# Shimly-2/DRL-on-robot-arm

Hardware: AMD Instinct MI355X
Metric: env-steps/sec at N parallel envs (rl_reach_env) (higher is better)
Workload: dtype f64

## Files before the change

### drl-on-robot-arm_amd/csrc/armenv_learner.h

```cpp
#pragma once
#include <hip/hip_runtime.h>
#include <stdint.h>

#include "armenv_math.h"

namespace armenv {
namespace learner {

constexpr int LRN_H = 256;
constexpr int LRN_A = 3;
constexpr int LRN_TM = 64, LRN_TN = 64, LRN_TK = 16;
constexpr int LRN_KSPLIT = 256;
constexpr int LRN_MAX_GEMMS = 6;
constexpr int LRN_MAX_TENSORS = 12;

struct Feat {
  const float *p0, *p1;
  int ld0, ld1, split, nf, aug;
  int64_t rows;
};

AE_DEV float feat_at(const Feat &F, int64_t r, int f) {
  if (r >= F.rows) return 0.f;
  if (f < F.split) return F.p0[r * F.ld0 + f];
  if (f < F.nf) return F.p1[r * F.ld1 + (f - F.split)];
  return (F.aug && f == F.nf) ? 1.f : 0.f;
}

enum { EPI_STORE = 0,
       EPI_BIAS_RELU = 1,
       EPI_MASK = 2,
       EPI_DRELU_W = 3 };

struct Gemm {
  Feat a, b;
  int ta, tb;
  int M, N;
  int64_t K, kchunk;
  int splits, tiles_m, tiles_n, first_block;
  float *C;
  int ldc;
  int64_t split_stride;
  int epi;
  const float *bias, *mask, *w;
  int ldm;
  float scale;
};

struct GemmList {
  Gemm g[LRN_MAX_GEMMS];
  int n;
};


AE_DEV float wave_sum(float x) {
#pragma unroll
  for (int o = 32; o >= 1; o >>= 1) x += __shfl_xor(x, o, 64);
  return x;
}

AE_DEV float4 row4(const float *p, int64_t b, int lane) { return reinterpret_cast<const float4 *>(p + b * LRN_H)[lane]; }
AE_DEV float dot4(float4 a, float4 b) { return a.x * b.x + a.y * b.y + a.z * b.z + a.w * b.w; }

AE_DEV void box_muller(uint32_t w0, uint32_t w1, float &z0, float &z1) {
  const float u1 = (float)((w0 >> 8) + 1u) * (1.0f / 16777216.0f);
  const float u2 = (float)(w1 >> 8) * (1.0f / 16777216.0f);
  const float r = sqrtf(-2.0f * logf(u1));
  float sn, cs;
  sincosf(6.283185307179586f * u2, &sn, &cs);
  z0 = r * cs;
  z1 = r * sn;
}


AE_DEV void head3(const float *h2, const float *W3, const float *b3, int64_t b, int lane, float (&u)[LRN_A]) {
  const float4 h = row4(h2, b, lane);
#pragma unroll
  for (int j = 0; j < LRN_A; ++j) u[j] = wave_sum(dot4(h, row4(W3, j, lane))) + b3[j];
}

AE_DEV float head1(float4 h, float4 w, const float *b3) { return wave_sum(dot4(h, w)) + b3[0]; }
AE_DEV float head1(const float *h2, const float *W3, const float *b3, int64_t b, int lane) {
  return head1(row4(h2, b, lane), row4(W3, 0, lane), b3);
}

AE_DEV void row_noise(const float *noise, uint64_t seed, uint64_t draw, float policy_noise, float noise_clip, int64_t b,
                      float (&nz)[LRN_A]) {
  float z[4];
  if (noise) {
#pragma unroll
    for (int j = 0; j < LRN_A; ++j) z[j] = noise[b * LRN_A + j];
  } else {
    uint32_t c[4] = {(uint32_t)b, (uint32_t)((uint64_t)b >> 32), (uint32_t)draw, (uint32_t)(draw >> 32)};
    philox4x32_10(c, (uint32_t)seed, (uint32_t)(seed >> 32));
    box_muller(c[0], c[1], z[0], z[1]);
    box_muller(c[2], c[3], z[2], z[3]);
  }
#pragma unroll
  for (int j = 0; j < LRN_A; ++j) nz[j] = fminf(fmaxf(z[j] * policy_noise, -noise_clip), noise_clip);
}

AE_DEV float proposal(float u, float nz, float bound) {
  const float v = tanhf(u) * bound + nz;
  return fminf(fmaxf(v, -bound), bound);
}

AE_DEV void store_action(const float (&u)[LRN_A], float bound, float *a, float *tanh_out, bool keep_tanh, int64_t b) {
#pragma unroll
  for (int j = 0; j < LRN_A; ++j) {
    const float th = tanhf(u[j]);
    if (keep_tanh) tanh_out[b * LRN_A + j] = th;
    a[b * LRN_A + j] = th * bound;
  }
}

AE_DEV void store_d2(float4 h, float4 w, float d3, float *d2, int64_t b, int lane) {
  float4 d;
  d.x = h.x > 0.f ? d3 * w.x : 0.f;
  d.y = h.y > 0.f ? d3 * w.y : 0.f;
  d.z = h.z > 0.f ? d3 * w.z : 0.f;
  d.w = h.w > 0.f ? d3 * w.w : 0.f;
  reinterpret_cast<float4 *>(d2 + b * LRN_H)[lane] = d;
}

struct ActorHeadArgs {
  int64_t B;
  const float *t_h2, *t_W3, *t_b3, *noise;
  uint64_t seed, draw;
  float bound, policy_noise, noise_clip;
  float *a2;
  int with_actor;
  const float *h2, *W3, *b3;
  float *a, *tanh_out;
};


struct CriticHeadArgs {
  int64_t B;
  float gamma, inv_b;
  const float *rewards;
  const uint8_t *dones;
  const float *t_h2[2], *t_W3[2], *t_b3[2];
  const float *h2[2], *W3[2], *b3[2];
  float *d3[2];
  float *d2[2];
  float *loss_rows;
};


struct DaddpgActorHeadArgs {
  int64_t B;
  float bound;
  const float *h2[3], *W3[3], *b3[3];
  float *a[3];
  float *tanh_out;
};

struct DaddpgCriticHeadArgs {
  int64_t B;
  float gamma, inv_b;
  const float *rewards;
  const uint8_t *dones;
  const float *t_h2[2];
  const float *t_W3, *t_b3;
  const float *h2, *W3, *b3;
  float *d3;
  float *d2;
  float *loss_rows;
};

struct Datd3ActorHeadArgs {
  int64_t B;
  float bound, policy_noise, noise_clip;
  const float *noise;
  uint64_t seed, draw;
  const float *t_h2[2], *t_W3[2], *t_b3[2];
  float *a2[2];
  const float *h2, *W3, *b3;
  float *a, *tanh_out;
};

struct Datd3CriticHeadArgs {
  int64_t B;
  float gamma, inv_b;
  int darc;
  float w_min, w_max, reg;
  const float *rewards;
  const uint8_t *dones;
  const float *t_h2[2], *t_W3[2], *t_b3[2];
  const float *h2, *W3, *b3;
  const float *o_h2, *o_W3, *o_b3;
  float *d3;
  float *d2;
  float *loss_rows;
};

struct ActorBackArgs {
  int64_t B;
  int in_dim;
  int state_dim;
  float bound;
  const float *dc1;
  const float *Wq1;
  const float *tanh_a;
  const float *h2, *W3;
  float *du;
  float *da2;
};


struct AdamTensor {
  float *p, *m, *v, *tp;
  const float *partial;
  int rows, cols, ldp, c0;
  int first;
};

struct AdamArgs {
  AdamTensor t[LRN_MAX_TENSORS];
  int n, total, splits;
  int64_t split_stride;
  float step_size, bc2_sqrt, beta1, beta2, eps, tau;
  int soft;
  const float *loss_rows;
  int loss_cols;
  float loss_w1;
  int64_t B;
  float inv_b;
  float *loss;
};


struct GemmStride {
  int64_t a0, a1, b0, b1;
  int64_t C, bias, mask, w;
};

struct GemmStrideList {
  GemmStride g[LRN_MAX_GEMMS];
};

struct HeadStride {
  int64_t ws, W3, b3, rows, noise;
};

struct ActorBackStride {
  int64_t ws, Wq1, W3;
};

#define LRN_POP 0
#include "armenv_learner_kernels.inc"
#undef LRN_POP
#define LRN_POP 1
#include "armenv_learner_kernels.inc"
#undef LRN_POP

}
}
```

### drl-on-robot-arm_amd/csrc/armenv_learner_kernels.inc

```
#if LRN_POP
#define LRN_KERNEL(name) name##_pop_kernel
#define LRN_POP_PARAM(decl) , decl
#define LRN_MEMBER(ptr, stride) ((ptr) + (int64_t)blockIdx.y * (stride))
#else
#define LRN_KERNEL(name) name##_kernel
#define LRN_POP_PARAM(decl)
#define LRN_MEMBER(ptr, stride) ptr
#endif

__global__ __launch_bounds__(256) void LRN_KERNEL(gemm)(GemmList L LRN_POP_PARAM(GemmStrideList S)) {
  __shared__ float As[LRN_TK][LRN_TM + 4];
  __shared__ float Bs[LRN_TK][LRN_TN + 4];
  int pi = 0;
  while (pi + 1 < L.n && (int)blockIdx.x >= L.g[pi + 1].first_block) ++pi;
#if LRN_POP
  Gemm G = L.g[pi];
  {
    const GemmStride &T = S.g[pi];
    const int64_t p = blockIdx.y;
    G.a.p0 += p * T.a0; G.a.p1 += p * T.a1;
    G.b.p0 += p * T.b0; G.b.p1 += p * T.b1;
    G.C += p * T.C; G.bias += p * T.bias; G.mask += p * T.mask; G.w += p * T.w;
  }
#else
  const Gemm &G = L.g[pi];
#endif
  int t = (int)blockIdx.x - G.first_block;
  const int tn = t % G.tiles_n;
  t /= G.tiles_n;
  const int tm = t % G.tiles_m;
  const int s = t / G.tiles_m;
  const int m0 = tm * LRN_TM, n0 = tn * LRN_TN;
  const int64_t kbeg = (int64_t)s * G.kchunk;
  const int64_t kend = kbeg + G.kchunk < G.K ? kbeg + G.kchunk : G.K;
  const int tid = threadIdx.x, lane = tid & 63, wave = tid >> 6;
  const int wm = (wave & 1) * 32, wn = (wave >> 1) * 32;
  typedef float f32x16 __attribute__((ext_vector_type(16)));
  f32x16 acc;
#pragma unroll
  for (int r = 0; r < 16; ++r) acc[r] = 0.f;

  for (int64_t k0 = kbeg; k0 < kend; k0 += LRN_TK) {
#pragma unroll
    for (int i = 0; i < LRN_TM * LRN_TK / 256; ++i) {
      const int e = tid + 256 * i;
      int mm, kk;
      if (G.ta) { mm = e % LRN_TM; kk = e / LRN_TM; } else { kk = e % LRN_TK; mm = e / LRN_TK; }
      const int64_t k = k0 + kk;
      float v = 0.f;
      if (k < kend) v = G.ta ? feat_at(G.a, k, m0 + mm) : feat_at(G.a, m0 + mm, (int)k);
      As[kk][mm] = v;
    }
#pragma unroll
    for (int i = 0; i < LRN_TN * LRN_TK / 256; ++i) {
      const int e = tid + 256 * i;
      int nn, kk;
      if (G.tb) { kk = e % LRN_TK; nn = e / LRN_TK; } else { nn = e % LRN_TN; kk = e / LRN_TN; }
      const int64_t k = k0 + kk;
      float v = 0.f;
      if (k < kend) v = G.tb ? feat_at(G.b, n0 + nn, (int)k) : feat_at(G.b, k, n0 + nn);
      Bs[kk][nn] = v;
    }
    __syncthreads();
#pragma unroll
    for (int kk = 0; kk < LRN_TK; kk += 2) {
      const float av = As[kk + (lane >> 5)][wm + (lane & 31)];
      const float bv = Bs[kk + (lane >> 5)][wn + (lane & 31)];
      acc = __builtin_amdgcn_mfma_f32_32x32x2f32(av, bv, acc, 0, 0, 0);
    }
    __syncthreads();
  }

  float *C = G.C + (int64_t)s * G.split_stride;
  const int n = n0 + wn + (lane & 31);
  if (n >= G.N) return;
#pragma unroll
  for (int r = 0; r < 16; ++r) {
    const int m = m0 + wm + (r & 3) + 8 * (r >> 2) + 4 * (lane >> 5);
    if (m >= G.M) continue;
    float v = acc[r];
    if (G.epi == EPI_BIAS_RELU) {
      v = v + G.bias[n];
      v = v > 0.f ? v : 0.f;
    } else if (G.epi == EPI_MASK) {
      v = G.mask[(int64_t)m * G.ldm + n] > 0.f ? v : 0.f;
    } else if (G.epi == EPI_DRELU_W) {
      v = (v + G.bias[n] > 0.f) ? G.scale * G.w[n] : 0.f;
    }
    C[(int64_t)m * G.ldc + n] = v;
  }
}

__global__ __launch_bounds__(256) void LRN_KERNEL(actor_head)(ActorHeadArgs P LRN_POP_PARAM(HeadStride S)) {
#if LRN_POP
  {
    const int64_t p = blockIdx.y;
    P.t_h2 += p * S.ws; P.a2 += p * S.ws; P.h2 += p * S.ws; P.a += p * S.ws; P.tanh_out += p * S.ws;
    P.t_W3 += p * S.W3; P.W3 += p * S.W3; P.t_b3 += p * S.b3; P.b3 += p * S.b3;
    if (P.noise) P.noise += p * S.noise;
    P.seed += (uint64_t)p;
  }
#endif
  const int lane = threadIdx.x & 63;
  const int64_t nb = (P.B + 3) / 4;
  const bool actor = (int64_t)blockIdx.x >= nb;
  const int64_t b = ((int64_t)blockIdx.x - (actor ? nb : 0)) * 4 + (threadIdx.x >> 6);
  if (b >= P.B) return;
  float u[LRN_A];
  head3(actor ? P.h2 : P.t_h2, actor ? P.W3 : P.t_W3, actor ? P.b3 : P.t_b3, b, lane, u);
  if (lane != 0) return;
  if (actor) {
    store_action(u, P.bound, P.a, P.tanh_out, true, b);
    return;
  }
  float nz[LRN_A];
  row_noise(P.noise, P.seed, P.draw, P.policy_noise, P.noise_clip, b, nz);
#pragma unroll
  for (int j = 0; j < LRN_A; ++j) P.a2[b * LRN_A + j] = proposal(u[j], nz[j], P.bound);
}

__global__ __launch_bounds__(256) void LRN_KERNEL(critic_head)(CriticHeadArgs P LRN_POP_PARAM(HeadStride S)) {
#if LRN_POP
  {
    const int64_t p = blockIdx.y;
    P.rewards += p * S.rows; P.dones += p * S.rows; P.loss_rows += p * S.ws;
#pragma unroll
    for (int i = 0; i < 2; ++i) {
      P.t_h2[i] += p * S.ws; P.h2[i] += p * S.ws; P.d3[i] += p * S.ws; P.d2[i] += p * S.ws;
      P.t_W3[i] += p * S.W3; P.W3[i] += p * S.W3; P.t_b3[i] += p * S.b3; P.b3[i] += p * S.b3;
    }
  }
#endif
  const int lane = threadIdx.x & 63;
  const int64_t b = (int64_t)blockIdx.x * 4 + (threadIdx.x >> 6);
  if (b >= P.B) return;
  float tq[2], q[2];
#pragma unroll
  for (int i = 0; i < 2; ++i) {
    tq[i] = head1(P.t_h2[i], P.t_W3[i], P.t_b3[i], b, lane);
    q[i] = head1(P.h2[i], P.W3[i], P.b3[i], b, lane);
  }
  const float notdone = 1.0f - (P.dones[b] ? 1.0f : 0.0f);
  const float target = P.rewards[b] + notdone * P.gamma * fminf(tq[0], tq[1]);
#pragma unroll
  for (int i = 0; i < 2; ++i) {
    const float e = q[i] - target;
    const float d3 = 2.0f * e * P.inv_b;
    if (lane == 0) {
      P.d3[i][b] = d3;
      P.loss_rows[2 * b + i] = e * e;
    }
    store_d2(row4(P.h2[i], b, lane), row4(P.W3[i], 0, lane), d3, P.d2[i], b, lane);
  }
}

__global__ __launch_bounds__(256) void LRN_KERNEL(daddpg_actor_head)(DaddpgActorHeadArgs P LRN_POP_PARAM(HeadStride S)) {
  const int lane = threadIdx.x & 63;
  const int64_t nb = (P.B + 3) / 4;
  const int k = (int)((int64_t)blockIdx.x / nb);
  const int64_t b = ((int64_t)blockIdx.x - k * nb) * 4 + (threadIdx.x >> 6);
  if (k > 2 || b >= P.B) return;
  float u[LRN_A];
  head3(LRN_MEMBER(P.h2[k], S.ws), LRN_MEMBER(P.W3[k], S.W3), LRN_MEMBER(P.b3[k], S.b3), b, lane, u);
  if (lane != 0) return;
  store_action(u, P.bound, LRN_MEMBER(P.a[k], S.ws), LRN_MEMBER(P.tanh_out, S.ws), k == 2, b);
}

__global__ __launch_bounds__(256) void LRN_KERNEL(daddpg_critic_head)(DaddpgCriticHeadArgs P LRN_POP_PARAM(HeadStride S)) {
#if LRN_POP
  {
    const int64_t p = blockIdx.y;
    P.rewards += p * S.rows; P.dones += p * S.rows;
    P.t_h2[0] += p * S.ws; P.t_h2[1] += p * S.ws; P.h2 += p * S.ws; P.d3 += p * S.ws; P.d2 += p * S.ws; P.loss_rows += p * S.ws;
    P.t_W3 += p * S.W3; P.W3 += p * S.W3; P.t_b3 += p * S.b3; P.b3 += p * S.b3;
  }
#endif
  const int lane = threadIdx.x & 63;
  const int64_t b = (int64_t)blockIdx.x * 4 + (threadIdx.x >> 6);
  if (b >= P.B) return;
  const float4 tw = row4(P.t_W3, 0, lane);
  const float tq0 = head1(row4(P.t_h2[0], b, lane), tw, P.t_b3);
  const float tq1 = head1(row4(P.t_h2[1], b, lane), tw, P.t_b3);
  const float4 h = row4(P.h2, b, lane), w = row4(P.W3, 0, lane);
  const float q = head1(h, w, P.b3);
  const float notdone = 1.0f - (P.dones[b] ? 1.0f : 0.0f);
  const float target = P.rewards[b] + notdone * P.gamma * fminf(tq0, tq1);
  const float e = q - target;
  const float d3 = 2.0f * e * P.inv_b;
  if (lane == 0) {
    P.d3[b] = d3;
    P.loss_rows[b] = e * e;
  }
  store_d2(h, w, d3, P.d2, b, lane);
}

__global__ __launch_bounds__(256) void LRN_KERNEL(datd3_actor_head)(Datd3ActorHeadArgs P LRN_POP_PARAM(HeadStride S)) {
#if LRN_POP
  {
    const int64_t p = blockIdx.y;
#pragma unroll
    for (int i = 0; i < 2; ++i) { P.t_h2[i] += p * S.ws; P.a2[i] += p * S.ws; P.t_W3[i] += p * S.W3; P.t_b3[i] += p * S.b3; }
    P.h2 += p * S.ws; P.a += p * S.ws; P.tanh_out += p * S.ws; P.W3 += p * S.W3; P.b3 += p * S.b3;
    if (P.noise) P.noise += p * S.noise;
    P.seed += (uint64_t)p;
  }
#endif
  const int lane = threadIdx.x & 63;
  const int64_t nb = (P.B + 3) / 4;
  const bool actor = (int64_t)blockIdx.x >= nb;
  const int64_t b = ((int64_t)blockIdx.x - (actor ? nb : 0)) * 4 + (threadIdx.x >> 6);
  if (b >= P.B) return;
  if (actor) {
    float u[LRN_A];
    head3(P.h2, P.W3, P.b3, b, lane, u);
    if (lane != 0) return;
    store_action(u, P.bound, P.a, P.tanh_out, true, b);
    return;
  }
  float u[2][LRN_A];
#pragma unroll
  for (int i = 0; i < 2; ++i) head3(P.t_h2[i], P.t_W3[i], P.t_b3[i], b, lane, u[i]);
  if (lane != 0) return;
  float nz[LRN_A];
  row_noise(P.noise, P.seed, P.draw, P.policy_noise, P.noise_clip, b, nz);
#pragma unroll
  for (int j = 0; j < LRN_A; ++j) {
#pragma unroll
    for (int i = 0; i < 2; ++i) P.a2[i][b * LRN_A + j] = proposal(u[i][j], nz[j], P.bound);
  }
}

__global__ __launch_bounds__(256) void LRN_KERNEL(datd3_critic_head)(Datd3CriticHeadArgs P LRN_POP_PARAM(HeadStride S)) {
#if LRN_POP
  {
    const int64_t p = blockIdx.y;
    P.rewards += p * S.rows; P.dones += p * S.rows;
#pragma unroll
    for (int i = 0; i < 2; ++i) { P.t_h2[i] += p * S.ws; P.t_W3[i] += p * S.W3; P.t_b3[i] += p * S.b3; }
    P.h2 += p * S.ws; P.d3 += p * S.ws; P.d2 += p * S.ws; P.loss_rows += p * S.ws; P.W3 += p * S.W3; P.b3 += p * S.b3;
    if (P.darc) { P.o_h2 += p * S.ws; P.o_W3 += p * S.W3; P.o_b3 += p * S.b3; }
  }
#endif
  const int lane = threadIdx.x & 63;
  const int64_t b = (int64_t)blockIdx.x * 4 + (threadIdx.x >> 6);
  if (b >= P.B) return;
  const float tq0 = head1(P.t_h2[0], P.t_W3[0], P.t_b3[0], b, lane);
  const float tq1 = head1(P.t_h2[1], P.t_W3[1], P.t_b3[1], b, lane);
  const float4 h = row4(P.h2, b, lane), w = row4(P.W3, 0, lane);
  const float q = head1(h, w, P.b3);
  float t = fminf(tq0, tq1);
  if (P.darc) t = P.w_min * t + P.w_max * t;
  const float notdone = 1.0f - (P.dones[b] ? 1.0f : 0.0f);
  const float target = P.rewards[b] + notdone * P.gamma * t;
  const float e = q - target;
  float d3 = 2.0f * e * P.inv_b;
  if (P.darc) {
    const float eo = q - head1(P.o_h2, P.o_W3, P.o_b3, b, lane);
    d3 += P.reg * (2.0f * eo * P.inv_b);
    if (lane == 0) {
      P.loss_rows[2 * b] = e * e;
      P.loss_rows[2 * b + 1] = eo * eo;
    }
  } else if (lane == 0) {
    P.loss_rows[b] = e * e;
  }
  if (lane == 0) P.d3[b] = d3;
  store_d2(h, w, d3, P.d2, b, lane);
}

__global__ __launch_bounds__(256) void LRN_KERNEL(actor_back)(ActorBackArgs P LRN_POP_PARAM(ActorBackStride S)) {
#if LRN_POP
  {
    const int64_t p = blockIdx.y;
    P.dc1 += p * S.ws; P.tanh_a += p * S.ws; P.h2 += p * S.ws; P.du += p * S.ws; P.da2 += p * S.ws;
    P.Wq1 += p * S.Wq1; P.W3 += p * S.W3;
  }
#endif
  const int lane = threadIdx.x & 63;
  const int64_t b = (int64_t)blockIdx.x * 4 + (threadIdx.x >> 6);
  if (b >= P.B) return;
  const float4 d = row4(P.dc1, b, lane);
  float du[LRN_A];
#pragma unroll
  for (int j = 0; j < LRN_A; ++j) {
    const float *w = P.Wq1 + P.state_dim + j;
    float4 wc;
    wc.x = w[(4 * lane + 0) * P.in_dim];
    wc.y = w[(4 * lane + 1) * P.in_dim];
    wc.z = w[(4 * lane + 2) * P.in_dim];
    wc.w = w[(4 * lane + 3) * P.in_dim];
    const float da = wave_sum(dot4(d, wc));
    const float th = P.tanh_a[b * LRN_A + j];
    du[j] = da * P.bound * (1.0f - th * th);
  }
  if (lane == 0) {
#pragma unroll
    for (int j = 0; j < LRN_A; ++j) P.du[b * LRN_A + j] = du[j];
  }
  const float4 h = row4(P.h2, b, lane);
  float4 w0 = row4(P.W3, 0, lane), w1 = row4(P.W3, 1, lane), w2 = row4(P.W3, 2, lane), o;
  o.x = h.x > 0.f ? du[0] * w0.x + du[1] * w1.x + du[2] * w2.x : 0.f;
  o.y = h.y > 0.f ? du[0] * w0.y + du[1] * w1.y + du[2] * w2.y : 0.f;
  o.z = h.z > 0.f ? du[0] * w0.z + du[1] * w1.z + du[2] * w2.z : 0.f;
  o.w = h.w > 0.f ? du[0] * w0.w + du[1] * w1.w + du[2] * w2.w : 0.f;
  reinterpret_cast<float4 *>(P.da2 + b * LRN_H)[lane] = o;
}

__global__ __launch_bounds__(256) void LRN_KERNEL(adam)(AdamArgs P LRN_POP_PARAM(int64_t ws_stride)) {
#if LRN_POP
  const int64_t member = blockIdx.y;
#define LRN_LOSS_ROWS (P.loss_rows + member * ws_stride)
#define LRN_LOSS (P.loss + member)
#else
#define LRN_LOSS_ROWS P.loss_rows
#define LRN_LOSS P.loss
#endif
  const int64_t e = (int64_t)blockIdx.x * 256 + threadIdx.x;
  const int64_t elem_blocks = ((int64_t)P.total + 255) / 256;
  if ((int64_t)blockIdx.x >= elem_blocks) {
    __shared__ float red[2][256];
    float s0 = 0.f, s1 = 0.f;
    if (P.loss_cols == 2) {
      for (int64_t b = threadIdx.x; b < P.B; b += 256) {
        s0 += LRN_LOSS_ROWS[2 * b];
        s1 += LRN_LOSS_ROWS[2 * b + 1];
      }
    } else {
      for (int64_t b = threadIdx.x; b < P.B; b += 256) s0 += LRN_LOSS_ROWS[b];
    }
    red[0][threadIdx.x] = s0;
    red[1][threadIdx.x] = s1;
    __syncthreads();
    for (int o = 128; o >= 1; o >>= 1) {
      if ((int)threadIdx.x < o) {
        red[0][threadIdx.x] += red[0][threadIdx.x + o];
        red[1][threadIdx.x] += red[1][threadIdx.x + o];
      }
      __syncthreads();
    }
    if (threadIdx.x == 0 && P.loss) LRN_LOSS[0] = P.loss_cols == 2 ? red[0][0] * P.inv_b + P.loss_w1 * (red[1][0] * P.inv_b) : red[0][0] * P.inv_b;
    return;
  }
  if (e >= P.total) return;
  int ti = 0;
  while (ti + 1 < P.n && e >= P.t[ti + 1].first) ++ti;
#if LRN_POP
  AdamTensor T = P.t[ti];
  {
    const int64_t own = member * ((int64_t)T.rows * T.cols);
    T.p += own; T.m += own; T.v += own; T.tp += own; T.partial += member * ws_stride;
  }
#else
  const AdamTensor &T = P.t[ti];
#endif
  const int i = (int)(e - T.first);
  const int r = i / T.cols, c = i % T.cols;
  const float *g_p = T.partial + (int64_t)r * T.ldp + T.c0 + c;
  float g = 0.f;
  for (int s = 0; s < P.splits; ++s) g += g_p[(int64_t)s * P.split_stride];
  const float m = P.beta1 * T.m[i] + (1.0f - P.beta1) * g;
  const float v = P.beta2 * T.v[i] + (1.0f - P.beta2) * g * g;
  T.m[i] = m;
  T.v[i] = v;
  const float p = T.p[i] - P.step_size * m / (sqrtf(v) / P.bc2_sqrt + P.eps);
  T.p[i] = p;
  if (P.soft) T.tp[i] = T.tp[i] * (1.0f - P.tau) + P.tau * p;
}

#undef LRN_LOSS_ROWS
#undef LRN_LOSS
#undef LRN_KERNEL
#undef LRN_MEMBER
#undef LRN_POP_PARAM
```

Before: 11.55 billion.

## Double-buffer learner GEMM LDS tiles with vectorized swizzled loads and TK=32

Rewrites the learner GEMM main loop so that global loads for the next K slice are issued into registers while MFMAs run on the current LDS buffer. Two LDS buffers remove the second barrier per iteration. Tile loads use float4 vector reads when the slice is whole and aligned, and LDS stores use an XOR swizzle to avoid bank conflicts. K tile depth grows from 16 to 32, and waves whose sub-tile lies outside M/N skip the MFMA work. The cost is more LDS and register pressure, plus more complex boundary handling.

New measurement: 11.53 billion (median of 2 runs). Within noise of the previous version (-0.1%).

```diff
diff --git a/drl-on-robot-arm_amd/csrc/armenv_learner.h b/drl-on-robot-arm_amd/csrc/armenv_learner.h
--- a/drl-on-robot-arm_amd/csrc/armenv_learner.h
+++ b/drl-on-robot-arm_amd/csrc/armenv_learner.h
@@ -9,7 +9,7 @@
 
 constexpr int LRN_H = 256;
 constexpr int LRN_A = 3;
-constexpr int LRN_TM = 64, LRN_TN = 64, LRN_TK = 16;
+constexpr int LRN_TM = 64, LRN_TN = 64, LRN_TK = 32;
 constexpr int LRN_KSPLIT = 256;
 constexpr int LRN_MAX_GEMMS = 6;
 constexpr int LRN_MAX_TENSORS = 12;
@@ -52,6 +52,58 @@
   int n;
 };
 
+static_assert(LRN_TM == 64 && LRN_TN == 64 && LRN_TK == 32, "slice_load / slice_store map 256 threads onto a 64 x 32 slice");
+
+AE_DEV int slice_swizzle(int kk) { return ((kk >> 2) & 7) << 2; }
+
+AE_DEV void slice_load(const Feat &F, int kfeat, int o0, int64_t k0, int64_t kend, int tid, float4 (&v)[2]) {
+  const int64_t r0 = kfeat ? o0 : k0, f0 = kfeat ? k0 : o0;
+  const int nr = kfeat ? 64 : LRN_TK, nf = kfeat ? LRN_TK : 64;
+  const int rr = kfeat ? tid >> 3 : tid >> 4, rstep = kfeat ? 32 : 16;
+  const int ff = kfeat ? 4 * (tid & 7) : 4 * (tid & 15);
+  const bool seg1 = f0 >= F.split;
+  const float *p = seg1 ? F.p1 : F.p0;
+  const int ld = seg1 ? F.ld1 : F.ld0;
+  const int64_t fs = seg1 ? f0 - F.split : f0, fend = seg1 ? F.nf : F.split;
+  const bool whole = k0 + LRN_TK <= kend && r0 + nr <= F.rows && f0 + nf <= fend;
+  const bool aligned = (((uintptr_t)p | (uintptr_t)ld | (uintptr_t)fs) & 3) == 0 && ((uintptr_t)p & 15) == 0;
+  if (whole && aligned) {
+#pragma unroll
+    for (int i = 0; i < 2; ++i) v[i] = *reinterpret_cast<const float4 *>(p + (r0 + rr + i * rstep) * ld + fs + ff);
+    return;
+  }
+#pragma unroll
+  for (int i = 0; i < 2; ++i) {
+    float e[4];
+#pragma unroll
+    for (int j = 0; j < 4; ++j) {
+      const int64_t r = r0 + rr + i * rstep, f = f0 + ff + j;
+      e[j] = (kfeat ? f : r) < kend ? feat_at(F, r, (int)f) : 0.f;
+    }
+    v[i] = make_float4(e[0], e[1], e[2], e[3]);
+  }
+}
+
+AE_DEV void slice_store(float *S, int kfeat, int tid, const float4 (&v)[2]) {
+  if (kfeat) {
+    const int k4 = 4 * (tid & 7);
+#pragma unroll
+    for (int i = 0; i < 2; ++i) {
+      const int o = ((tid >> 3) + 32 * i) ^ k4;
+      S[(k4 + 0) * 64 + o] = v[i].x;
+      S[(k4 + 1) * 64 + o] = v[i].y;
+      S[(k4 + 2) * 64 + o] = v[i].z;
+      S[(k4 + 3) * 64 + o] = v[i].w;
+    }
+  } else {
+#pragma unroll
+    for (int i = 0; i < 2; ++i) {
+      const int kk = (tid >> 4) + 16 * i;
+      *reinterpret_cast<float4 *>(S + kk * 64 + ((4 * (tid & 15)) ^ slice_swizzle(kk))) = v[i];
+    }
+  }
+}
+
 
 AE_DEV float wave_sum(float x) {
 #pragma unroll
diff --git a/drl-on-robot-arm_amd/csrc/armenv_learner_kernels.inc b/drl-on-robot-arm_amd/csrc/armenv_learner_kernels.inc
--- a/drl-on-robot-arm_amd/csrc/armenv_learner_kernels.inc
+++ b/drl-on-robot-arm_amd/csrc/armenv_learner_kernels.inc
@@ -9,8 +9,7 @@
 #endif
 
 __global__ __launch_bounds__(256) void LRN_KERNEL(gemm)(GemmList L LRN_POP_PARAM(GemmStrideList S)) {
-  __shared__ float As[LRN_TK][LRN_TM + 4];
-  __shared__ float Bs[LRN_TK][LRN_TN + 4];
+  __shared__ __attribute__((aligned(16))) float lds[2][2][LRN_TK * 64];
   int pi = 0;
   while (pi + 1 < L.n && (int)blockIdx.x >= L.g[pi + 1].first_block) ++pi;
 #if LRN_POP
@@ -35,41 +34,50 @@
   const int64_t kend = kbeg + G.kchunk < G.K ? kbeg + G.kchunk : G.K;
   const int tid = threadIdx.x, lane = tid & 63, wave = tid >> 6;
   const int wm = (wave & 1) * 32, wn = (wave >> 1) * 32;
+  const bool live = m0 + wm < G.M && n0 + wn < G.N;
   typedef float f32x16 __attribute__((ext_vector_type(16)));
   f32x16 acc;
 #pragma unroll
   for (int r = 0; r < 16; ++r) acc[r] = 0.f;
 
-  for (int64_t k0 = kbeg; k0 < kend; k0 += LRN_TK) {
-#pragma unroll
-    for (int i = 0; i < LRN_TM * LRN_TK / 256; ++i) {
-      const int e = tid + 256 * i;
-      int mm, kk;
-      if (G.ta) { mm = e % LRN_TM; kk = e / LRN_TM; } else { kk = e % LRN_TK; mm = e / LRN_TK; }
-      const int64_t k = k0 + kk;
-      float v = 0.f;
-      if (k < kend) v = G.ta ? feat_at(G.a, k, m0 + mm) : feat_at(G.a, m0 + mm, (int)k);
-      As[kk][mm] = v;
-    }
-#pragma unroll
-    for (int i = 0; i < LRN_TN * LRN_TK / 256; ++i) {
-      const int e = tid + 256 * i;
-      int nn, kk;
-      if (G.tb) { kk = e % LRN_TK; nn = e / LRN_TK; } else { nn = e % LRN_TN; kk = e / LRN_TN; }
-      const int64_t k = k0 + kk;
-      float v = 0.f;
-      if (k < kend) v = G.tb ? feat_at(G.b, n0 + nn, (int)k) : feat_at(G.b, k, n0 + nn);
-      Bs[kk][nn] = v;
-    }
+  float4 ra[2], rb[2];
+  slice_load(G.a, !G.ta, m0, kbeg, kend, tid, ra);
+  slice_load(G.b, G.tb, n0, kbeg, kend, tid, rb);
+  slice_store(lds[0][0], !G.ta, tid, ra);
+  slice_store(lds[0][1], G.tb, tid, rb);
+  __syncthreads();
+  int buf = 0;
+  for (int64_t k0 = kbeg;; k0 += LRN_TK, buf ^= 1) {
+    const int64_t k1 = k0 + LRN_TK;
+    if (k1 < kend) {
+      slice_load(G.a, !G.ta, m0, k1, kend, tid, ra);
+      slice_load(G.b, G.tb, n0, k1, kend, tid, rb);
+    }
+    if (live) {
+      const float *As = lds[buf][0] + (lane >> 5) * 64, *Bs = lds[buf][1] + (lane >> 5) * 64;
+      const int am = wm + (lane & 31), bn = wn + (lane & 31);
+      if (k1 <= kend) {
+#pragma unroll
+        for (int kk = 0; kk < LRN_TK; kk += 2) {
+          const float av = As[kk * 64 + (am ^ slice_swizzle(kk))];
+          const float bv = Bs[kk * 64 + (bn ^ slice_swizzle(kk))];
+          acc = __builtin_amdgcn_mfma_f32_32x32x2f32(av, bv, acc, 0, 0, 0);
+        }
+      } else {
+        const int nk = (int)(kend - k0);
+        for (int kk = 0; kk < nk; kk += 2) {
+          const float av = As[kk * 64 + (am ^ slice_swizzle(kk))];
+          const float bv = Bs[kk * 64 + (bn ^ slice_swizzle(kk))];
+          acc = __builtin_amdgcn_mfma_f32_32x32x2f32(av, bv, acc, 0, 0, 0);
+        }
+      }
+    }
+    if (k1 >= kend) break;
+    slice_store(lds[buf ^ 1][0], !G.ta, tid, ra);
+    slice_store(lds[buf ^ 1][1], G.tb, tid, rb);
     __syncthreads();
-#pragma unroll
-    for (int kk = 0; kk < LRN_TK; kk += 2) {
-      const float av = As[kk + (lane >> 5)][wm + (lane & 31)];
-      const float bv = Bs[kk + (lane >> 5)][wn + (lane & 31)];
-      acc = __builtin_amdgcn_mfma_f32_32x32x2f32(av, bv, acc, 0, 0, 0);
-    }
-    __syncthreads();
-  }
+  }
+  if (!live) return;
 
   float *C = G.C + (int64_t)s * G.split_stride;
   const int n = n0 + wn + (lane & 31);
```
